# MuMuJun97/semantic_slam_mapping

Measured on AMD Instinct MI355X. Metric: frames/sec semantic-mapping, 640x480 RGB-D, higher is better.
Workload: dtype u8; 1 GPU; configs[1]: synthetic 640x480 RGB-D + precomputed 12-class masks, 1k frames per GPU, ORB 1000 kp/frame, 5 ref frames, leaf 0.10 m; frames_per_gpu=1000, frames_all_gpus=1000, batch_frames=250, matcher_halo_frames=0, parallelism=single GPU

## Files before the change

### semantic_slam_mapping_amd/csrc/kernels_match.hip

```cpp
#include "ssm_internal.h"

#define MT 512
#define TCH 1024

#define QPL 2
__device__ __forceinline__ uint32_t bcnt_acc(uint32_t x, uint32_t acc)
{
    uint32_t r;
    asm("v_bcnt_u32_b32 %0, %1, %2" : "=v"(r) : "v"(x), "v"(acc));
    return r;
}
__device__ __forceinline__ uint32_t umed3(uint32_t a, uint32_t b, uint32_t c)
{
    uint32_t r;
    asm("v_med3_u32 %0, %1, %2, %3" : "=v"(r) : "v"(a), "v"(b), "v"(c));
    return r;
}
template <int T>
__device__ __forceinline__ void match_pair(const uint8_t* __restrict__ q, int nq, const uint8_t* __restrict__ t, int nt,
                                           double ratio, int cap, ssm_dmatch* __restrict__ out, int32_t* __restrict__ nout,
                                           int32_t* __restrict__ knn_idx, int32_t* __restrict__ knn_dist,
                                           int qb = 0, int qe = -1, int32_t* __restrict__ pend = nullptr, int role = 0)
{
    __shared__ uint4 tr[TCH * 2];
    __shared__ int wcnt[T / 64];
    __shared__ int base;
    const int tid = threadIdx.x, lane = tid & 63, wv = tid >> 6;
    if (qe < 0) qe = nq;
    if (tid == 0) base = role == 2 ? qb : 0;
    for (int q0 = qb; q0 < qe; q0 += T * QPL) {
        uint4 a[QPL], b[QPL]; uint32_t k0[QPL], k1[QPL];
#pragma unroll
        for (int u = 0; u < QPL; u++) {
            const int qi = q0 + u * T + tid;
            a[u] = make_uint4(0, 0, 0, 0); b[u] = a[u]; k0[u] = 0xFFFFFFFFu; k1[u] = 0xFFFFFFFFu;
            if (qi < qe) { const uint4* p = reinterpret_cast<const uint4*>(q + (size_t)qi * 32); a[u] = p[0]; b[u] = p[1]; }
        }
        for (int t0 = 0; t0 < nt; t0 += TCH) {
            const int m = min(TCH, nt - t0);
            __syncthreads();
            for (int i = tid; i < m * 2; i += T) tr[i] = reinterpret_cast<const uint4*>(t + (size_t)t0 * 32)[i];
            __syncthreads();
            auto one_train = [&](int j) {
                const uint4 x = tr[2 * j], y = tr[2 * j + 1];
#pragma unroll
                for (int u = 0; u < QPL; u++) {
                    uint32_t d = bcnt_acc(a[u].x ^ x.x, 0u);
                    d = bcnt_acc(a[u].y ^ x.y, d); d = bcnt_acc(a[u].z ^ x.z, d); d = bcnt_acc(a[u].w ^ x.w, d);
                    d = bcnt_acc(b[u].x ^ y.x, d); d = bcnt_acc(b[u].y ^ y.y, d); d = bcnt_acc(b[u].z ^ y.z, d); d = bcnt_acc(b[u].w ^ y.w, d);
                    const uint32_t key = (d << 16) | (uint32_t)(t0 + j);
                    k1[u] = umed3(key, k0[u], k1[u]);
                    k0[u] = min(key, k0[u]);
                }
            };
            const int m4 = m & ~3;
            for (int j = 0; j < m4; j += 4) {
#pragma unroll
                for (int jj = 0; jj < 4; jj++) one_train(j + jj);
            }
            for (int j = m4; j < m; j++) one_train(j);
        }
#pragma unroll
        for (int u = 0; u < QPL; u++) {
            const int qi = q0 + u * T + tid;
            const int d0 = k0[u] >> 16, i0 = k0[u] & 0xFFFF, d1 = k1[u] >> 16, i1 = k1[u] & 0xFFFF;
            if (knn_idx && qi < qe) { knn_idx[2*qi] = i0; knn_idx[2*qi+1] = i1; knn_dist[2*qi] = d0; knn_dist[2*qi+1] = d1; }
            const bool keep = (qi < qe) && ((double)(float)d0 < ratio * (double)(float)d1);
            const unsigned long long bal = __ballot(keep);
            __syncthreads();
            if (lane == 0) wcnt[wv] = __popcll(bal);
            __syncthreads();
            int off = base;
            for (int w = 0; w < wv; w++) off += wcnt[w];
            if (keep) {
                const int k = off + __popcll(bal & ((1ull << lane) - 1ull));
                if (out && k < cap) { ssm_dmatch mm; mm.queryIdx = qi; mm.trainIdx = i0; mm.imgIdx = 0; mm.distance = (float)d0; out[k] = mm; }
            }
            __syncthreads();
            if (tid == 0) { int s = 0; for (int w = 0; w < T / 64; w++) s += wcnt[w]; base += s; }
        }
    }
    __syncthreads();
    if (role == 0) { if (tid == 0 && nout) *nout = base; return; }
    __shared__ int other;
    const int split = role == 1 ? qe : qb, mine = base - (role == 2 ? qb : 0);
    if (tid == 0) {
        __builtin_amdgcn_fence(__ATOMIC_RELEASE, "agent");
        asm volatile("s_waitcnt vmcnt(0)" ::: "memory");
        other = __hip_atomic_exchange(pend, mine, __ATOMIC_RELAXED, __HIP_MEMORY_SCOPE_AGENT);
        if (other >= 0) { __builtin_amdgcn_fence(__ATOMIC_ACQUIRE, "agent"); asm volatile("s_waitcnt vmcnt(0)" ::: "memory"); }
    }
    __syncthreads();
    if (other < 0) return;
    const int n0 = role == 1 ? mine : other, n1 = role == 1 ? other : mine;
    if (n0 != split) {
        uint4* o = reinterpret_cast<uint4*>(out);
        for (int i0 = 0; i0 < n1; i0 += T) {
            const int i = i0 + tid;
            uint4 v = make_uint4(0, 0, 0, 0);
            if (i < n1) v = o[split + i];
            __syncthreads();
            if (i < n1) o[n0 + i] = v;
            __syncthreads();
        }
    }
    if (tid == 0 && nout) *nout = n0 + n1;
}

__global__ void __launch_bounds__(MT)
match_pairs_kernel(const uint8_t* __restrict__ desc, const MatchPair* __restrict__ pairs, double ratio, int cap,
                   ssm_dmatch* __restrict__ out, int32_t* __restrict__ nout, int32_t* __restrict__ knn_idx, int32_t* __restrict__ knn_dist)
{
    const MatchPair p = pairs[blockIdx.x];
    match_pair<MT>(desc + (size_t)p.qoff * 32, p.nq, desc + (size_t)p.toff * 32, p.nt, ratio, cap,
               out ? out + (size_t)p.out_slot * cap : nullptr, nout ? nout + p.out_slot : nullptr, knn_idx, knn_dist);
}
hipError_t k_match_pairs(const uint8_t* desc, const MatchPair* pairs, int npairs, double ratio, int cap,
                         ssm_dmatch* out, int32_t* nout, int32_t* knn_idx, int32_t* knn_dist, hipStream_t s)
{
    match_pairs_kernel<<<npairs, MT, 0, s>>>(desc, pairs, ratio, cap, out, nout, knn_idx, knn_dist);
    return hipGetLastError();
}

__global__ void __launch_bounds__(MT / 2)
match_seq_kernel(const uint8_t* __restrict__ desc, const int32_t* __restrict__ nkp, int f0, int R, int hist, double ratio, int cap,
                 ssm_dmatch* __restrict__ out, int32_t* __restrict__ nout, int32_t* __restrict__ pend)
{
    const int f = f0 + blockIdx.y, r = blockIdx.x >> 1, half = blockIdx.x & 1;
    const int cur = hist + f, ref = cur - R + r;
    const int slot = f * R + r;
    const int nq = ref >= 0 ? nkp[ref] : -1, nt = nkp[cur];
    if (nq < 0 || nt < 2) { if (threadIdx.x == 0 && half == 0) nout[slot] = -1; return; }
    const int split = min(nq, (((nq + 1) >> 1) + 63) & ~63);
    match_pair<MT / 2>(desc + (size_t)ref * cap * 32, nq, desc + (size_t)cur * cap * 32, nt, ratio, cap,
                       out + (size_t)slot * cap, nout + slot, nullptr, nullptr, half ? split : 0, half ? nq : split, pend + blockIdx.y * R + r, half + 1);
}
hipError_t k_match_seq(const uint8_t* desc, const int32_t* nkp, int f0, int n, int R, int hist, double ratio, int cap,
                       ssm_dmatch* out, int32_t* nout, int32_t* pend, hipStream_t s)
{
    hipError_t e = hipMemsetAsync(pend, 0xFF, sizeof(int32_t) * (size_t)n * R, s);
    if (e != hipSuccess) return e;
    match_seq_kernel<<<dim3(2 * R, n), MT / 2, 0, s>>>(desc, nkp, f0, R, hist, ratio, cap, out, nout, pend);
    return hipGetLastError();
}

typedef int v4i __attribute__((ext_vector_type(4)));
typedef int v8i __attribute__((ext_vector_type(8)));
typedef float v16f __attribute__((ext_vector_type(16)));
typedef __attribute__((address_space(3))) void* lds_ptr_t;
#define MM_QB 256
#define MM_DB SSM_MATCH_DESC_BYTES
#define MM_KS 4
#define MM_TILE (32 * MM_DB)
#ifndef MM_ABLATE
#define MM_ABLATE 0
#endif

__global__ void __launch_bounds__(256)
match_expand_kernel(const uint8_t* __restrict__ desc, const int32_t* __restrict__ nkp, int row0, int cap, int capT,
                    uint8_t* __restrict__ eq, uint8_t* __restrict__ et)
{
    const int row = row0 + blockIdx.y;
    const int i = blockIdx.x * 256 + threadIdx.x;
    if (i >= capT * 8) return;
    const int r = i & 31, c = (i >> 5) & 7, d = (i >> 8) * 32 + r;
    uint32_t bits = 0;
    if (d < nkp[row]) bits = *reinterpret_cast<const uint32_t*>(desc + ((size_t)row * cap + d) * 32 + 4 * c);
    uint32_t q[4], t[4];
#pragma unroll
    for (int k = 0; k < 4; k++) {
        uint32_t v = (bits >> (8 * k)) & 255u;
        v = (v | (v << 12)) & 0x000F000Fu;
        v = (v | (v << 6)) & 0x03030303u;
        v = (v | (v << 3)) & 0x11111111u;
        q[k] = (v << 3) + 0x22222222u;
        t[k] = (v << 3) ^ 0xAAAAAAAAu;
    }
    const size_t o = (size_t)row * capT * MM_DB + (size_t)i * 16;
    *reinterpret_cast<uint4*>(eq + o) = make_uint4(q[0], q[1], q[2], q[3]);
    *reinterpret_cast<uint4*>(et + o) = make_uint4(t[0], t[1], t[2], t[3]);
}

__device__ __forceinline__ void mm_merge2(uint32_t& a0, uint32_t& a1, uint32_t b0, uint32_t b1)
{
    const uint32_t m = max(a0, b0);
    a0 = min(a0, b0);
    a1 = min(min(m, a1), b1);
}
__device__ __forceinline__ void mm_track(const v16f& acc, uint32_t t32, uint32_t& g0, uint32_t& g1)
{
    float l0 = __builtin_fminf(acc[0], acc[1]), l1 = __builtin_fmaxf(acc[0], acc[1]);
#pragma unroll
    for (int i = 2; i < 16; i++) { l1 = __builtin_amdgcn_fmed3f(acc[i], l0, l1); l0 = __builtin_fminf(acc[i], l0); }
    const uint32_t k0 = (uint32_t)l0, k1 = (uint32_t)l1;
    const uint32_t G0 = ((k0 >> 5) << 16) | ((k0 & 31u) | t32), G1 = ((k1 >> 5) << 16) | ((k1 & 31u) | t32);
    mm_merge2(g0, g1, G0, G1);
}

__global__ void __launch_bounds__(256, 2)
match_mfma_kernel(const uint8_t* __restrict__ eq, const uint8_t* __restrict__ et, const int32_t* __restrict__ nkp,
                  int f0, int n, int R, int hist, int capT, int qblocks, int frames_per_xcd, uint2* __restrict__ knn)
{
    __shared__ __attribute__((aligned(16))) uint4 ring0[MM_TILE / 16];
    __shared__ __attribute__((aligned(16))) uint4 ring1[MM_TILE / 16];
    __shared__ __attribute__((aligned(16))) uint4 ring2[MM_TILE / 16];
    __shared__ __attribute__((aligned(16))) uint4 ring3[MM_TILE / 16];
    const int Y = R * qblocks, xcd = blockIdx.x & 7, j = blockIdx.x >> 3;
    const int frame = xcd * frames_per_xcd + j / Y, y = j % Y;
    if (frame >= n) return;
    const int r = y / qblocks, qb = y - r * qblocks;
    const int f = f0 + frame, cur = hist + f, ref = cur - R + r;
    const int nq = ref >= 0 ? nkp[ref] : -1, nt = nkp[cur];
    if (nq < 0 || nt < 2 || qb * MM_QB >= nq) return;
    const int tid = threadIdx.x, lane = tid & 63, wv = tid >> 6, h = lane >> 5;
    const int q0 = qb * MM_QB + wv * 64;
    v4i b[2][MM_KS];
    {
        const uint4* qp = reinterpret_cast<const uint4*>(eq + ((size_t)ref * capT + q0) * MM_DB) + lane;
#pragma unroll
        for (int u = 0; u < 2; u++)
#pragma unroll
            for (int s = 0; s < MM_KS; s++) {
                uint4 v = make_uint4(0, 0, 0, 0);
                if (q0 + u * 32 < capT) v = qp[(u * MM_TILE + s * 1024) / 16];
                b[u][s] = v4i{(int)v.x, (int)v.y, (int)v.z, (int)v.w};
            }
    }
    v16f cc;
#pragma unroll
    for (int i = 0; i < 16; i++) cc[i] = (float)(4096 + (i & 3) + 8 * (i >> 2) + 4 * h);
    const int ntile = (nt + 31) >> 5;
    uint32_t g0[2] = {0xFFFFFFFFu, 0xFFFFFFFFu}, g1[2] = {0xFFFFFFFFu, 0xFFFFFFFFu};
    const auto rsT = __builtin_amdgcn_make_buffer_rsrc((void*)(et + (size_t)cur * capT * MM_DB), 0, (unsigned)capT * MM_DB, 0x00020000);
    const int wvu = __builtin_amdgcn_readfirstlane(wv);
    auto dma = [&](int T, uint4* ring) {
        if (MM_ABLATE & 4) return;
        const unsigned o = (unsigned)min(T, ntile - 1) * MM_TILE + (unsigned)(wvu * 64 + lane) * 16u;
        __builtin_amdgcn_raw_ptr_buffer_load_lds(rsT, (lds_ptr_t)&ring[wvu * 64], 16, o, 0, 0, 0);
    };
    auto frags = [&](const uint4* buf, v4i (&a)[MM_KS]) {
#pragma unroll
        for (int s = 0; s < MM_KS; s++) { const uint4 v = buf[s * 64 + lane]; a[s] = v4i{(int)v.x, (int)v.y, (int)v.z, (int)v.w}; }
    };
    auto mfma4 = [](const v4i& a, const v4i& bq, const v16f& c) {
        const v8i a8 = {a[0], a[1], a[2], a[3], 0, 0, 0, 0}, b8 = {bq[0], bq[1], bq[2], bq[3], 0, 0, 0, 0};
        return __builtin_amdgcn_mfma_scale_f32_32x32x64_f8f6f4(a8, b8, c, 4, 4, 0, 0x83838383, 0, 0x7F7F7F7F);
    };
    auto issue = [&](const v4i (&a)[MM_KS], v16f& x0, v16f& x1) {
        if (MM_ABLATE & 8) { x0 = cc; x1 = cc; for (int s = 0; s < MM_KS; s++) { x0[s] += (float)a[s][0]; x1[s] += (float)a[s][1]; } return; }
        x0 = mfma4(a[0], b[0][0], cc);
        x1 = mfma4(a[0], b[1][0], cc);
#pragma unroll
        for (int s = 1; s < MM_KS; s++) {
            x0 = mfma4(a[s], b[0][s], x0);
            x1 = mfma4(a[s], b[1][s], x1);
        }
    };
    auto interleave = [&]() {
#pragma unroll
        for (int i = 0; i < 2 * MM_KS; i++) { __builtin_amdgcn_sched_group_barrier(0x008, 1, 0); __builtin_amdgcn_sched_group_barrier(0x002, 12, 0); }
    };
    auto track = [&](const v16f& x0, const v16f& x1, int T) {
        if (MM_ABLATE & 1) { g0[0] = min(g0[0], __float_as_uint(x0[0])); g0[1] = min(g0[1], __float_as_uint(x1[0])); return; }
        mm_track(x0, (uint32_t)T << 5, g0[0], g1[0]); mm_track(x1, (uint32_t)T << 5, g0[1], g1[1]);
    };
    auto track_last = [&](v16f x0, v16f x1, int T) {
        const int valid = nt - T * 32;
#pragma unroll
        for (int i = 0; i < 16; i++) if ((i & 3) + 8 * (i >> 2) + 4 * h >= valid) { x0[i] = 1048576.0f; x1[i] = 1048576.0f; }
        track(x0, x1, T);
    };
#define MM_STEP(T_, rd_, wr_, acur, anxt, xn0, xn1, TRACK) { \
        __builtin_amdgcn_s_waitcnt((MM_ABLATE & 4) ? 0x007F : 0x0072);     \
        if (!(MM_ABLATE & 2)) __builtin_amdgcn_s_barrier();               \
        frags(rd_, anxt); \
        dma((T_) + 4, wr_); \
        __builtin_amdgcn_sched_barrier(0); \
        issue(acur, xn0, xn1); TRACK; interleave(); \
        __builtin_amdgcn_sched_barrier(0); }
    v16f A0, A1, B0, B1;
    v4i aA[MM_KS], aB[MM_KS];
    dma(0, ring0); dma(1, ring1); dma(2, ring2); dma(3, ring3);
    if (!(MM_ABLATE & 4)) __builtin_amdgcn_s_waitcnt(0x0F73);
    if (!(MM_ABLATE & 2)) __builtin_amdgcn_s_barrier();
    frags(ring0, aA);
    MM_STEP(0, ring1, ring0, aA, aB, A0, A1, (void)0)
    int T = 1;
    for (; T + 3 < ntile; T += 4) {
        MM_STEP(T, ring2, ring1, aB, aA, B0, B1, track(A0, A1, T - 1))
        MM_STEP(T + 1, ring3, ring2, aA, aB, A0, A1, track(B0, B1, T))
        MM_STEP(T + 2, ring0, ring3, aB, aA, B0, B1, track(A0, A1, T + 1))
        MM_STEP(T + 3, ring1, ring0, aA, aB, A0, A1, track(B0, B1, T + 2))
    }
    if (T < ntile) MM_STEP(T, ring2, ring1, aB, aA, B0, B1, track(A0, A1, T - 1))
    if (T + 1 < ntile) MM_STEP(T + 1, ring3, ring2, aA, aB, A0, A1, track(B0, B1, T))
    if (T + 2 < ntile) MM_STEP(T + 2, ring0, ring3, aB, aA, B0, B1, track(A0, A1, T + 1))
#undef MM_STEP
    if ((ntile - 1) & 1) track_last(B0, B1, ntile - 1); else track_last(A0, A1, ntile - 1);
    __builtin_amdgcn_s_waitcnt(0x0070);
#pragma unroll
    for (int u = 0; u < 2; u++) {
        const uint32_t o0 = __shfl_xor(g0[u], 32), o1 = __shfl_xor(g1[u], 32);
        const uint32_t m = max(g0[u], o0);
        g0[u] = min(g0[u], o0);
        g1[u] = min(min(m, g1[u]), o1);
    }
    const uint32_t k0 = h ? g0[1] : g0[0], k1 = h ? g1[1] : g1[0];
    const int qi = q0 + lane;
    const int slot = f * R + r;
    if (qi < nq) knn[(size_t)slot * capT + qi] = make_uint2(k0, k1);
}

__global__ void __launch_bounds__(256)
match_compact_kernel(const uint2* __restrict__ knn, const int32_t* __restrict__ nkp, int f0, int R, int hist, int capT, double ratio, int cap,
                     ssm_dmatch* __restrict__ out, int32_t* __restrict__ nout)
{
    __shared__ int wcnt[4];
    const int slot = (f0 + blockIdx.x / R) * R + blockIdx.x % R;
    const int cur = hist + f0 + blockIdx.x / R, ref = cur - R + blockIdx.x % R;
    const int nq = ref >= 0 ? nkp[ref] : -1, nt = nkp[cur];
    const int tid = threadIdx.x, lane = tid & 63, wv = tid >> 6;
    if (nq < 0 || nt < 2) { if (tid == 0) nout[slot] = -1; return; }
    const uint2* kk = knn + (size_t)slot * capT;
    ssm_dmatch* o = out + (size_t)slot * cap;
    int base = 0;
    for (int q0 = 0; q0 < nq; q0 += 256) {
        const int qi = q0 + tid;
        uint2 k = make_uint2(0, 0);
        if (qi < nq) k = kk[qi];
        const int d0 = k.x >> 16, i0 = k.x & 0xFFFF, d1 = k.y >> 16;
        const bool keep = (qi < nq) && ((double)(float)d0 < ratio * (double)(float)d1);
        const unsigned long long bal = __ballot(keep);
        if (lane == 0) wcnt[wv] = __popcll(bal);
        __syncthreads();
        int off = base;
        for (int w = 0; w < wv; w++) off += wcnt[w];
        if (keep) {
            const int kpos = off + __popcll(bal & ((1ull << lane) - 1ull));
            if (kpos < cap) { ssm_dmatch mm; mm.queryIdx = qi; mm.trainIdx = i0; mm.imgIdx = 0; mm.distance = (float)d0; o[kpos] = mm; }
        }
        base += wcnt[0] + wcnt[1] + wcnt[2] + wcnt[3];
        __syncthreads();
    }
    if (tid == 0) nout[slot] = base;
}
hipError_t k_match_expand(const uint8_t* desc, const int32_t* nkp, int row0, int nrows, int cap, int capT, uint8_t* eq, uint8_t* et, hipStream_t s)
{
    if (nrows <= 0) return hipSuccess;
    match_expand_kernel<<<dim3((capT * 8 + 255) / 256, nrows), 256, 0, s>>>(desc, nkp, row0, cap, capT, eq, et);
    return hipGetLastError();
}
hipError_t k_match_seq_mfma(const uint8_t* eq, const uint8_t* et, const int32_t* nkp, int f0, int n, int R, int hist, double ratio, int cap, int capT,
                            void* knn, ssm_dmatch* out, int32_t* nout, hipStream_t s)
{
    const int qblocks = (capT + MM_QB - 1) / MM_QB;
    const int fpx = (n + 7) >> 3;
    match_mfma_kernel<<<8 * fpx * R * qblocks, 256, 0, s>>>(eq, et, nkp, f0, n, R, hist, capT, qblocks, fpx, reinterpret_cast<uint2*>(knn));
    match_compact_kernel<<<n * R, 256, 0, s>>>(reinterpret_cast<const uint2*>(knn), nkp, f0, R, hist, capT, ratio, cap, out, nout);
    return hipGetLastError();
}
```

Measured before the change: 185,500 frames/s.

## Encode global train index into MFMA distance keys to cheapen top-2 tracking

Adds a GLOBAL_KEYS variant of the MFMA Hamming matcher. The accumulator bias and scale exponent are chosen so that each float result already encodes distance<<kb plus the global train index. The running top-2 is then tracked directly in float with a rebasing offset per tile, replacing the per-tile integer key construction and merge. This roughly halves the VALU work interleaved with MFMAs (sched group count 12 to 6). It relies on float exactness within the chosen key range and is enabled only when capT fits.

```diff
diff --git a/semantic_slam_mapping_amd/csrc/kernels_match.hip b/semantic_slam_mapping_amd/csrc/kernels_match.hip
--- a/semantic_slam_mapping_amd/csrc/kernels_match.hip
+++ b/semantic_slam_mapping_amd/csrc/kernels_match.hip
@@ -1,4 +1,5 @@
 #include "ssm_internal.h"
+#include <type_traits>
 
 #define MT 512
 #define TCH 1024
@@ -181,6 +182,16 @@
     *reinterpret_cast<uint4*>(et + o) = make_uint4(t[0], t[1], t[2], t[3]);
 }
 
+__device__ __forceinline__ void mm_track_global(const v16f& acc, float& l0, float& l1)
+{
+    l0 -= 32.0f; l1 -= 32.0f;
+#pragma unroll
+    for (int i = 0; i < 16; i += 2) {
+        const float m = __builtin_amdgcn_fmed3f(l0, acc[i], acc[i + 1]);
+        l0 = __builtin_fminf(__builtin_fminf(l0, acc[i]), acc[i + 1]);
+        l1 = __builtin_fminf(l1, m);
+    }
+}
 __device__ __forceinline__ void mm_merge2(uint32_t& a0, uint32_t& a1, uint32_t b0, uint32_t b1)
 {
     const uint32_t m = max(a0, b0);
@@ -197,9 +208,10 @@
     mm_merge2(g0, g1, G0, G1);
 }
 
+template <bool GLOBAL_KEYS>
 __global__ void __launch_bounds__(256, 2)
 match_mfma_kernel(const uint8_t* __restrict__ eq, const uint8_t* __restrict__ et, const int32_t* __restrict__ nkp,
-                  int f0, int n, int R, int hist, int capT, int qblocks, int frames_per_xcd, uint2* __restrict__ knn)
+                  int f0, int n, int R, int hist, int capT, int qblocks, int frames_per_xcd, int kb, uint32_t scaleA, uint2* __restrict__ knn)
 {
     __shared__ __attribute__((aligned(16))) uint4 ring0[MM_TILE / 16];
     __shared__ __attribute__((aligned(16))) uint4 ring1[MM_TILE / 16];
@@ -228,9 +240,11 @@
     }
     v16f cc;
 #pragma unroll
-    for (int i = 0; i < 16; i++) cc[i] = (float)(4096 + (i & 3) + 8 * (i >> 2) + 4 * h);
+    for (int i = 0; i < 16; i++) cc[i] = (float)((128 << kb) + (i & 3) + 8 * (i >> 2) + 4 * h);
     const int ntile = (nt + 31) >> 5;
-    uint32_t g0[2] = {0xFFFFFFFFu, 0xFFFFFFFFu}, g1[2] = {0xFFFFFFFFu, 0xFFFFFFFFu};
+    using run_t = std::conditional_t<GLOBAL_KEYS, float, uint32_t>;
+    const run_t rinit = GLOBAL_KEYS ? (run_t)3.0e38f : (run_t)0xFFFFFFFFu;
+    run_t r0[2] = {rinit, rinit}, r1[2] = {rinit, rinit};
     const auto rsT = __builtin_amdgcn_make_buffer_rsrc((void*)(et + (size_t)cur * capT * MM_DB), 0, (unsigned)capT * MM_DB, 0x00020000);
     const int wvu = __builtin_amdgcn_readfirstlane(wv);
     auto dma = [&](int T, uint4* ring) {
@@ -242,9 +256,9 @@
 #pragma unroll
         for (int s = 0; s < MM_KS; s++) { const uint4 v = buf[s * 64 + lane]; a[s] = v4i{(int)v.x, (int)v.y, (int)v.z, (int)v.w}; }
     };
-    auto mfma4 = [](const v4i& a, const v4i& bq, const v16f& c) {
+    auto mfma4 = [scaleA](const v4i& a, const v4i& bq, const v16f& c) {
         const v8i a8 = {a[0], a[1], a[2], a[3], 0, 0, 0, 0}, b8 = {bq[0], bq[1], bq[2], bq[3], 0, 0, 0, 0};
-        return __builtin_amdgcn_mfma_scale_f32_32x32x64_f8f6f4(a8, b8, c, 4, 4, 0, 0x83838383, 0, 0x7F7F7F7F);
+        return __builtin_amdgcn_mfma_scale_f32_32x32x64_f8f6f4(a8, b8, c, 4, 4, 0, (int)scaleA, 0, 0x7F7F7F7F);
     };
     auto issue = [&](const v4i (&a)[MM_KS], v16f& x0, v16f& x1) {
         if (MM_ABLATE & 8) { x0 = cc; x1 = cc; for (int s = 0; s < MM_KS; s++) { x0[s] += (float)a[s][0]; x1[s] += (float)a[s][1]; } return; }
@@ -258,16 +272,22 @@
     };
     auto interleave = [&]() {
 #pragma unroll
-        for (int i = 0; i < 2 * MM_KS; i++) { __builtin_amdgcn_sched_group_barrier(0x008, 1, 0); __builtin_amdgcn_sched_group_barrier(0x002, 12, 0); }
+        for (int i = 0; i < 2 * MM_KS; i++) { __builtin_amdgcn_sched_group_barrier(0x008, 1, 0); __builtin_amdgcn_sched_group_barrier(0x002, GLOBAL_KEYS ? 6 : 12, 0); }
     };
     auto track = [&](const v16f& x0, const v16f& x1, int T) {
-        if (MM_ABLATE & 1) { g0[0] = min(g0[0], __float_as_uint(x0[0])); g0[1] = min(g0[1], __float_as_uint(x1[0])); return; }
-        mm_track(x0, (uint32_t)T << 5, g0[0], g1[0]); mm_track(x1, (uint32_t)T << 5, g0[1], g1[1]);
+        if constexpr (GLOBAL_KEYS) {
+            if (MM_ABLATE & 1) { r0[0] = __builtin_fminf(r0[0], x0[0]); r0[1] = __builtin_fminf(r0[1], x1[0]); return; }
+            mm_track_global(x0, r0[0], r1[0]); mm_track_global(x1, r0[1], r1[1]);
+        } else {
+            if (MM_ABLATE & 1) { r0[0] = min(r0[0], __float_as_uint(x0[0])); r0[1] = min(r0[1], __float_as_uint(x1[0])); return; }
+            mm_track(x0, (uint32_t)T << 5, r0[0], r1[0]); mm_track(x1, (uint32_t)T << 5, r0[1], r1[1]);
+        }
     };
     auto track_last = [&](v16f x0, v16f x1, int T) {
         const int valid = nt - T * 32;
-#pragma unroll
-        for (int i = 0; i < 16; i++) if ((i & 3) + 8 * (i >> 2) + 4 * h >= valid) { x0[i] = 1048576.0f; x1[i] = 1048576.0f; }
+        const float masked = GLOBAL_KEYS ? 1.0e30f : 1048576.0f;
+#pragma unroll
+        for (int i = 0; i < 16; i++) if ((i & 3) + 8 * (i >> 2) + 4 * h >= valid) { x0[i] = masked; x1[i] = masked; }
         track(x0, x1, T);
     };
 #define MM_STEP(T_, rd_, wr_, acur, anxt, xn0, xn1, TRACK) { \
@@ -298,14 +318,26 @@
 #undef MM_STEP
     if ((ntile - 1) & 1) track_last(B0, B1, ntile - 1); else track_last(A0, A1, ntile - 1);
     __builtin_amdgcn_s_waitcnt(0x0070);
-#pragma unroll
-    for (int u = 0; u < 2; u++) {
-        const uint32_t o0 = __shfl_xor(g0[u], 32), o1 = __shfl_xor(g1[u], 32);
-        const uint32_t m = max(g0[u], o0);
-        g0[u] = min(g0[u], o0);
-        g1[u] = min(min(m, g1[u]), o1);
-    }
-    const uint32_t k0 = h ? g0[1] : g0[0], k1 = h ? g1[1] : g1[0];
+    uint32_t k0, k1;
+    if constexpr (GLOBAL_KEYS) {
+#pragma unroll
+        for (int u = 0; u < 2; u++) {
+            const float o0 = __shfl_xor(r0[u], 32), o1 = __shfl_xor(r1[u], 32);
+            const float m = __builtin_fmaxf(r0[u], o0);
+            r0[u] = __builtin_fminf(r0[u], o0);
+            r1[u] = __builtin_fminf(__builtin_fminf(m, r1[u]), o1);
+        }
+        const float back = 32.0f * (float)(ntile - 1);
+        const uint32_t ga = (uint32_t)((h ? r0[1] : r0[0]) + back), gb = (uint32_t)((h ? r1[1] : r1[0]) + back), im = (1u << kb) - 1u;
+        k0 = ((ga >> kb) << 16) | (ga & im); k1 = ((gb >> kb) << 16) | (gb & im);
+    } else {
+#pragma unroll
+        for (int u = 0; u < 2; u++) {
+            const uint32_t o0 = __shfl_xor(r0[u], 32), o1 = __shfl_xor(r1[u], 32);
+            mm_merge2(r0[u], r1[u], o0, o1);
+        }
+        k0 = h ? r0[1] : r0[0]; k1 = h ? r1[1] : r1[0];
+    }
     const int qi = q0 + lane;
     const int slot = f * R + r;
     if (qi < nq) knn[(size_t)slot * capT + qi] = make_uint2(k0, k1);
@@ -355,7 +387,12 @@
 {
     const int qblocks = (capT + MM_QB - 1) / MM_QB;
     const int fpx = (n + 7) >> 3;
-    match_mfma_kernel<<<8 * fpx * R * qblocks, 256, 0, s>>>(eq, et, nkp, f0, n, R, hist, capT, qblocks, fpx, reinterpret_cast<uint2*>(knn));
+    const bool global_keys = capT <= 32768;
+    int kb = 5;
+    if (global_keys) while ((1 << kb) < capT) kb++;
+    const uint32_t scaleA = (uint32_t)(127 + kb - 1) * 0x01010101u;
+    if (global_keys) match_mfma_kernel<true><<<8 * fpx * R * qblocks, 256, 0, s>>>(eq, et, nkp, f0, n, R, hist, capT, qblocks, fpx, kb, scaleA, reinterpret_cast<uint2*>(knn));
+    else match_mfma_kernel<false><<<8 * fpx * R * qblocks, 256, 0, s>>>(eq, et, nkp, f0, n, R, hist, capT, qblocks, fpx, kb, scaleA, reinterpret_cast<uint2*>(knn));
     match_compact_kernel<<<n * R, 256, 0, s>>>(reinterpret_cast<const uint2*>(knn), nkp, f0, R, hist, capT, ratio, cap, out, nout);
     return hipGetLastError();
 }
```

Result: no change. 187,200 frames/s, median of 4 (+0.9%).
